# SCUT-CCNL/3DSIFT

Measured on AMD Instinct MI355X. Metric: Mvoxels/s end-to-end KpSiftAlgorithm on 512^3 fp32, higher is better.
Workload: dtype f32

## Files before the change

### 3dsift_amd/csrc/context.hip

```cpp
#include <float.h>
#include <math.h>
#include <stdlib.h>
#include <string.h>

#include <algorithm>
#include <atomic>
#include <mutex>
#include <thread>

#include "ctx_internal.h"

#pragma clang fp contract(off)

namespace s3d {

static thread_local std::string g_last_error;
void set_last_error(const std::string &s) { g_last_error = s; }

int set_device(int device) {
	int n = 0;
	if (hipGetDeviceCount(&n) != hipSuccess || n <= 0) {
		set_last_error("no HIP device visible: this library has no CPU fallback");
		return SIFT3D_ERR_NO_DEVICE;
	}
// ... 96 lines not shown
	}
}

extern "C" const char *sift3d_last_error(void) { return g_last_error.c_str(); }

extern "C" int sift3d_destroy(sift3d_handle c) {
	if (!c) return SIFT3D_OK;
	hipSetDevice(c->device);
	c->pending = false;
	if (c->uploader.joinable()) c->uploader.join();
	if (c->up_stream) { hipStreamSynchronize(c->up_stream); hipStreamDestroy(c->up_stream); c->up_stream = nullptr; }
	if (c->stream) hipStreamSynchronize(c->stream);
	if (c->own_stream && c->own_stream != c->stream) hipStreamSynchronize(c->own_stream);
	free_lists(c);
	if (!c->ext_arena) hipFree(c->arena);
	hipFree(c->in_own);
	hipFree(c->d_peer);
	hipFree(c->d_words);
	if (c->h_words) (void)hipHostFree(c->h_words);
	hipFree(c->d_slots_part);
	hipFree(c->det.masks); hipFree(c->det.block_counts); hipFree(c->det.block_offsets);
	hipFree(c->d_masks2); hipFree(c->d_counts2); hipFree(c->d_offsets2);
	if (c->ev_det_fork) hipEventDestroy(c->ev_det_fork);
	if (c->ev_det_join) hipEventDestroy(c->ev_det_join);
	if (c->ev_det_fork2) hipEventDestroy(c->ev_det_fork2);
	if (c->ev_det_join2) hipEventDestroy(c->ev_det_join2);
	hipFree(c->d_levels); hipFree(c->d_luts); hipFree(c->d_lutpool);
	for (auto &e : c->ev) if (e) hipEventDestroy(e);
	for (auto &e : c->ev_seed) if (e) hipEventDestroy(e);
	for (auto &e : c->ev_done) if (e) hipEventDestroy(e);
	if (c->ev_fork) hipEventDestroy(c->ev_fork);
	for (size_t o = 1; o < c->ostream.size(); o++) if (c->ostream[o] && c->ostream[o] != c->stream && c->ostream[o] != c->own_stream) hipStreamDestroy(c->ostream[o]);
	if (c->cstream) hipStreamDestroy(c->cstream);
	if (c->own_stream) hipStreamDestroy(c->own_stream);
	delete c;
	return SIFT3D_OK;
}

static int octaves_of(int nx, int ny, int nz) {
	const int mn = std::min(nx, std::min(ny, nz));
	return std::max(0, (int)log2f((float)mn) - 3 + 1);
}

void plan_pyramid(sift3d_ctx *c, int noct_total) {
	c->noct = noct_total >= 0 ? std::max(0, noct_total - c->octave_base) : octaves_of(c->nx, c->ny, c->nz);
	if (c->slab) c->noct = std::min(c->noct, 1);
	c->ng = c->p.num_kp_levels + 3;
	c->nd = c->p.num_kp_levels + 2;
	c->gss.assign((size_t)c->noct * c->ng, Level());
	c->dog.assign((size_t)c->noct * c->nd, Level());
	const double sigma0 = (double)c->p.sigma_default * pow(2.0, -1.0 / 3.0);
	for (int pyr = 0; pyr < 2; pyr++) {
		const int interval = pyr ? c->nd : c->ng;
		std::vector<Level> &P = pyr ? c->dog : c->gss;
		int nx = c->nx, ny = c->ny, nz = c->nz;
		float u = (float)(1 << c->octave_base);
		for (int o = 0; o < c->noct; o++) {
			for (int s = 0; s < interval; s++) {
				Level &L = P[(size_t)o * interval + s];
				L.nx = nx; L.ny = ny; L.nz = nz; L.unit = u;
				const double scale_factor = pow(2.0, (double)(o + c->octave_base) + (double)s / (double)c->p.num_kp_levels);
				L.scale = (float)(scale_factor * sigma0);
				if (c->slab) { L.bz = c->own1 - c->own0 + 2 * c->halo; L.zoff = c->own0 - c->halo; }
			}
			nx /= 2; ny /= 2; nz /= 2;
			u *= 2;
		}
	}
}

int upload_luts(sift3d_ctx *c, const std::vector<WinLut> &luts, std::vector<float> &pool) {
	if (pool.empty()) pool.push_back(-1.0f);
	if (c->d_luts) { S3D_HIP(hipFree(c->d_luts)); c->d_luts = nullptr; }
	if (c->d_lutpool) { S3D_HIP(hipFree(c->d_lutpool)); c->d_lutpool = nullptr; }
	S3D_HIP(hipMalloc(&c->d_luts, sizeof(WinLut) * luts.size()));
	S3D_HIP(hipMalloc(&c->d_lutpool, sizeof(float) * pool.size()));
	S3D_HIP(hipMemcpy(c->d_luts, luts.data(), sizeof(WinLut) * luts.size(), hipMemcpyHostToDevice));
	S3D_HIP(hipMemcpy(c->d_lutpool, pool.data(), sizeof(float) * pool.size(), hipMemcpyHostToDevice));
	return SIFT3D_OK;
}

std::vector<WinLut> blank_luts(const sift3d_ctx *c) {
	std::vector<WinLut> luts((size_t)std::max(1, c->noct + c->octave_base) * 8 * 2);
	for (auto &l : luts) { l.off = 0; l.len = 0; l.nin = -1; l.radius = 0; l.sigma = 0; l.fix_scale = 1.0f; l.wsum = 1.0f; l.list_off = -1; l.list_R = 0; }
	return luts;
}

static int build_luts(sift3d_ctx *c) {
	std::vector<WinLut> luts = blank_luts(c);
	std::vector<float> pool;
	for (int o = 0; o < c->noct; o++)
		for (int lv = 1; lv <= c->p.num_kp_levels && lv < 8; lv++) {
			const Level &D = c->dog[(size_t)o * c->nd + lv];
			const float u = D.unit, scale = D.scale;
			for (int which = 0; which < 2; which++) {
				float sigma, radius;
				if (which == 0) { sigma = 1.5f * scale; radius = sigma * 3.0f; }
				else { sigma = scale * 7.071067812f; radius = 2.0f * sigma; }
				if (!append_lut(pool, luts[((size_t)(o + c->octave_base) * 8 + lv) * 2 + which], which, sigma, radius, u, scale)) c->desc_lut_lds = false;
			}
		}
	return upload_luts(c, luts, pool);
}

static size_t al64(size_t n) { return (n + 63) & ~(size_t)63; }

size_t arena_floats_of(const sift3d_ctx *c) {
	size_t total = c->in_own ? 0 : al64(c->in.n());
	if (!c->slab) for (int o = 0; o < c->noct; o++) total += 2 * al64(c->gss[(size_t)o * c->ng].n());
	for (auto &L : c->gss) total += al64(L.n());
	for (auto &L : c->dog) total += al64(L.n());
	return total;
}

int create_common(sift3d_handle *out, const CreateCfg &cfg, const sift3d_params *params, int device) {
	*out = nullptr;
	if (cfg.nx <= 0 || cfg.ny <= 0 || cfg.nz <= 0) { set_last_error("bad dimensions"); return SIFT3D_ERR_ARG; }
	int rc = set_device(device);
	if (rc) return rc;
	sift3d_ctx *c = new sift3d_ctx();
	c->device = device;
	if (params) c->p = *params; else sift3d_default_params(&c->p);
	sift3d_default_detect_options(&c->dopt);
	if (c->p.num_kp_levels < 1 || c->p.num_kp_levels > 5) { delete c; set_last_error("num_kp_levels must be in [1,5]"); return SIFT3D_ERR_ARG; }
	c->nx = cfg.nx; c->ny = cfg.ny; c->nz = cfg.nz;
	c->octave_base = cfg.octave_base; c->seeded = cfg.seeded;
	c->slab = cfg.slab; c->own0 = cfg.z0; c->own1 = cfg.z1; c->halo = cfg.halo;
	c->use_fused = !hook(SIFT3D_HOOK_SEPARABLE);
	plan_pyramid(c, cfg.noct_total);
	c->in.nx = cfg.nx; c->in.ny = cfg.ny; c->in.nz = cfg.nz; c->in.unit = (float)(1 << c->octave_base); c->in.scale = 1.f;
	if (c->slab) { c->in.bz = c->own1 - c->own0 + 2 * c->halo; c->in.zoff = c->own0 - c->halo; }
	if (c->seeded) c->in.bz = 1;
	for (auto &L : c->gss) if ((size_t)L.nx * L.ny * L.planes() >= ((size_t)1 << 31)) { delete c; set_last_error("level too large for int32 voxel indices"); return SIFT3D_ERR_ARG; }

	std::vector<float> sig;
	float base_sigma;
	level_sigmas(c->p, sig, base_sigma);
	c->taps.resize(c->ng);
	bool ok = build_taps(base_sigma, c->base_taps);
	for (int i = 1; i < c->ng; i++) ok = ok && build_taps(sig[i], c->taps[i]);
	if (!ok) { delete c; set_last_error("Gaussian kernel wider than the supported 129 taps"); return SIFT3D_ERR_ARG; }

#define CHECKED(call) do { hipError_t e_ = (call); if (e_ != hipSuccess) { set_last_error(std::string(#call) + ": " + hipGetErrorString(e_)); sift3d_destroy(c); return SIFT3D_ERR_HIP; } } while (0)
	CHECKED(hipStreamCreateWithFlags(&c->stream, hipStreamNonBlocking));
	for (auto &e : c->ev) CHECKED(hipEventCreate(&e));
	CHECKED(hipEventCreateWithFlags(&c->ev_fork, hipEventDisableTiming));
	c->ostream.assign((size_t)std::max(1, c->noct), nullptr);
	c->ev_seed.assign(c->ostream.size(), nullptr);
	c->ev_done.assign(c->ostream.size(), nullptr);
	c->own_stream = c->stream;
	c->ostream[0] = c->stream;
	if (cfg.host_volume && !cfg.ext_arena && !c->slab && !c->seeded) {
		const size_t V0 = c->in.n();
		CHECKED(hipMalloc(&c->in_own, sizeof(float) * al64(V0)));
		CHECKED(hipStreamCreateWithFlags(&c->up_stream, hipStreamNonBlocking));
		const float *vol = cfg.host_volume;
		c->uploader = std::thread([c, vol, V0, device] {
			int r = set_device(device);
			if (r == SIFT3D_OK) r = staged_h2d(c->in_own, vol, sizeof(float) * V0, device, c->up_stream);
			if (r != SIFT3D_OK) c->upload_err = sift3d_last_error();
			c->upload_rc = r;
		});
	}
	const bool one_stream = hook(SIFT3D_HOOK_ONE_STREAM) != 0;
	for (size_t o = 0; o < c->ostream.size(); o++) {
		if (o > 0 && one_stream) c->ostream[o] = c->stream;
		else if (o > 0) {
// ... 734 lines not shown
```

### 3dsift_amd/csrc/kernels_orient.hip

```cpp
#include <float.h>

#include "sift3d_internal.h"

namespace s3d {

__device__ __forceinline__ float wave_sum(float v) {
#pragma unroll
	for (int o = 32; o > 0; o >>= 1) v = v + __shfl_xor(v, o, 64);
	return v;
}

__device__ __forceinline__ void win_bounds(float c, float rad, float u, int n, int &lo, int &hi) {
	int s = (int)floorf(c - __fdiv_rn(rad, u));
	lo = s > 1 ? s : 1;
	int e = (int)ceilf(c + __fdiv_rn(rad, u));
	hi = e < (n - 2) ? e : n - 2;
}

__device__ void eig_sym3(const double A[9], double w[3], double V[9]) {
	double a[9];
#pragma unroll
	for (int i = 0; i < 9; i++) { a[i] = A[i]; V[i] = (i % 4 == 0) ? 1.0 : 0.0; }
	for (int sweep = 0; sweep < 64; sweep++) {
		const double off = fabs(a[1]) + fabs(a[2]) + fabs(a[5]);
		const double diag = fabs(a[0]) + fabs(a[4]) + fabs(a[8]);
		if (off <= 1e-300 || off <= 1e-22 * diag) break;
#pragma unroll
		for (int pq = 0; pq < 3; pq++) {
			const int p = (pq == 2) ? 1 : 0, q = (pq == 0) ? 1 : 2;
			const double apq = a[3 * p + q];
			if (apq == 0.0) continue;
			const double theta = (a[4 * q] - a[4 * p]) / (2.0 * apq);
			const double t = (theta >= 0 ? 1.0 : -1.0) / (fabs(theta) + sqrt(theta * theta + 1.0));
			const double c = 1.0 / sqrt(t * t + 1.0), s = t * c;
#pragma unroll
			for (int k = 0; k < 3; k++) {
				const double akp = a[3 * k + p], akq = a[3 * k + q];
				a[3 * k + p] = c * akp - s * akq;
				a[3 * k + q] = s * akp + c * akq;
			}
#pragma unroll
			for (int k = 0; k < 3; k++) {
				const double apk = a[3 * p + k], aqk = a[3 * q + k];
				a[3 * p + k] = c * apk - s * aqk;
				a[3 * q + k] = s * apk + c * aqk;
			}
#pragma unroll
			for (int k = 0; k < 3; k++) {
				const double vkp = V[3 * k + p], vkq = V[3 * k + q];
				V[3 * k + p] = c * vkp - s * vkq;
				V[3 * k + q] = s * vkp + c * vkq;
			}
		}
	}
	w[0] = a[0]; w[1] = a[4]; w[2] = a[8];
#pragma unroll
	for (int j = 0; j < 3; j++) {
		const double n = sqrt(V[j] * V[j] + V[3 + j] * V[3 + j] + V[6 + j] * V[6 + j]);
		V[j] /= n; V[3 + j] /= n; V[6 + j] /= n;
	}
}

__device__ __forceinline__ float dot3f(const float *a, const float *b) { return a[0] * b[0] + a[1] * b[1] + a[2] * b[2]; }

__device__ int finish_orientation(DevKp &kp, const float T6[6], const float w3[3], float max_eig_ratio, float corner_thresh, bool *near = nullptr) {
	bool nr = false;
	float T[9] = {T6[0], T6[1], T6[2], T6[1], T6[3], T6[4], T6[2], T6[4], T6[5]};
#pragma unroll
	for (int i = 0; i < 9; i++) kp.st[i] = T[i];
	kp.win[0] = w3[0]; kp.win[1] = w3[1]; kp.win[2] = w3[2];
	const float gg = dot3f(w3, w3);
	nr = fabsf(gg - 1E-10f) <= 1E-13f;
	if (near) *near = nr;
	if (gg < 1E-10f) return -1;

	double A[9], wv[3], V[9];
#pragma unroll
	for (int i = 0; i < 9; i++) A[i] = (double)T[i];
	eig_sym3(A, wv, V);
	float val[3], vec[3][3];
#pragma unroll
	for (int j = 0; j < 3; j++) {
		val[j] = (float)wv[j];
		vec[j][0] = (float)V[j]; vec[j][1] = (float)V[3 + j]; vec[j][2] = (float)V[6 + j];
	}
#define S3D_CSWAP(i, j)                                                                   \
	if (val[j] < val[i]) {                                                                \
		float tv = val[i]; val[i] = val[j]; val[j] = tv;                                  \
		for (int c = 0; c < 3; c++) { float t2 = vec[i][c]; vec[i][c] = vec[j][c]; vec[j][c] = t2; } \
	}
	S3D_CSWAP(0, 1) S3D_CSWAP(1, 2) S3D_CSWAP(0, 1)
#undef S3D_CSWAP
#pragma unroll
	for (int j = 0; j < 3; j++) {
		kp.eigvalue[j] = val[j];
		kp.eigvector[3 * j] = vec[j][0]; kp.eigvector[3 * j + 1] = vec[j][1]; kp.eigvector[3 * j + 2] = vec[j][2];
	}
	const float r01 = fabsf(__fdiv_rn(val[0], val[1])), r12 = fabsf(__fdiv_rn(val[1], val[2]));
	nr = nr || fabsf(r01 - max_eig_ratio) <= 1e-4f || fabsf(r12 - max_eig_ratio) <= 1e-4f || !(r01 == r01) || !(r12 == r12);
	if (near) *near = nr;
	if (r01 > max_eig_ratio || r12 > max_eig_ratio) return -2;
	if ((double)fabsf(val[0] - val[1]) < DBL_EPSILON || (double)fabsf(val[0] - val[2]) < DBL_EPSILON ||
	    (double)fabsf(val[2] - val[1]) < DBL_EPSILON)
		return -2;

	const float d_norm = __fsqrt_rn(dot3f(w3, w3));
	float corner = FLT_MAX;
	for (int i = 2; i > 0; i--) {
		const float d = dot3f(vec[i], w3);
		const float q_norm = __fsqrt_rn(dot3f(vec[i], vec[i]));
		const float cos_ang = __fdiv_rn(d, d_norm * q_norm);
		const float a = fabsf(cos_ang);
		corner = corner < a ? corner : a;
		const float sgn = d > 0.0f ? 1.0f : -1.0f;
		vec[i][0] *= sgn; vec[i][1] *= sgn; vec[i][2] *= sgn;
	}
	nr = nr || fabsf(corner - corner_thresh) <= 1e-4f;
	if (near) *near = nr;
	if (corner < corner_thresh) return -3;
	if (near) *near = true;
	const float *v1 = vec[2], *v2 = vec[1];
	float vr[3];
	vr[0] = v1[1] * v2[2] - v1[2] * v2[1];
	vr[1] = v1[2] * v2[0] - v1[0] * v2[2];
	vr[2] = v1[0] * v2[1] - v1[1] * v2[0];
	kp.rot[0] = v1[0]; kp.rot[1] = v2[0]; kp.rot[2] = vr[0];
	kp.rot[3] = v1[1]; kp.rot[4] = v2[1]; kp.rot[5] = vr[1];
	kp.rot[6] = v1[2]; kp.rot[7] = v2[2]; kp.rot[8] = vr[2];
	return 1;
}

#ifndef S3D_ORI_UN
#define S3D_ORI_UN 2
#endif
constexpr int kTileW = 28, kTileH = 27;
constexpr int kTilePc = ((kTileW / 4) * kTileH + 63) / 64;
typedef float f4o __attribute__((ext_vector_type(4), aligned(4)));
constexpr int kOriLut = 256;

constexpr int kTermPitch = 68;
template <bool EXACT>
__global__ void __launch_bounds__(256) k_orient(DevKp *__restrict__ kps, int *__restrict__ codes, const unsigned *__restrict__ d_count, unsigned cap,
                                                const LevelRef *__restrict__ levels, const WinLut *__restrict__ luts,
                                                const float *__restrict__ lutpool, float max_eig, float corner, int part_rank,
                                                int part_world, const int *__restrict__ redo_list, const unsigned *__restrict__ redo_count) {
	__shared__ __attribute__((aligned(16))) float s_tile[4 * 3 * kTileW * kTileH];
	__shared__ float s_wlut[4 * kOriLut];
	__shared__ __attribute__((aligned(16))) float s_terms[EXACT ? 4 * 9 * kTermPitch : 4];
	const unsigned count = min(d_count[0], cap);
	const int lane = threadIdx.x & 63;
	const unsigned wave = blockIdx.x * (blockDim.x >> 6) + (threadIdx.x >> 6);
	const unsigned nwaves = gridDim.x * (blockDim.x >> 6);
	const unsigned pw = part_world > 1 ? (unsigned)part_world : 1u, pr = part_world > 1 ? (unsigned)part_rank : 0u;
	if (!EXACT && pw > 1)
		for (unsigned k = blockIdx.x * blockDim.x + threadIdx.x; k < count; k += gridDim.x * blockDim.x)
			if (k % pw != pr) { kps[k].code = 0; codes[k] = 0; }
	const unsigned owned = EXACT ? min(redo_count[0], cap) : (count > pr ? (count - pr + pw - 1) / pw : 0u);
	float *tb = &s_terms[EXACT ? (threadIdx.x >> 6) * 9 * kTermPitch : 0];
	for (unsigned j = wave; j < owned; j += nwaves) {
		const unsigned k = EXACT ? (unsigned)redo_list[j] : j * pw + pr;
		const int cxi = kps[k].x, cyi = kps[k].y, czi = kps[k].z;
		const int li = kps[k].octave * 8 + kps[k].level;
		const LevelRef L = levels[li];
		const WinLut lut = luts[li * 2 + 0];
		const float *__restrict__ wtab = lutpool + lut.off;
		const float u = L.unit, inv_u = __fdiv_rn(1.0f, u);
		int x0, x1, y0, y1, z0, z1;
		win_bounds((float)cxi, lut.radius, u, L.nx, x0, x1);
		win_bounds((float)cyi, lut.radius, u, L.ny, y0, y1);
		win_bounds((float)czi, lut.radius, u, L.nz, z0, z1);
		const int wx = x1 - x0 + 1, wy = y1 - y0 + 1;
		const int plane = (wx > 0 && wy > 0) ? wx * wy : 0;
		const float inv_wx = 1.0f / (float)(wx > 0 ? wx : 1);
		const size_t sy = (size_t)L.nx, sz = (size_t)L.nx * L.ny;
		const gfloat_p Ld = as_global(L.d);
		float t00 = 0.f, t01 = 0.f, t02 = 0.f, t11 = 0.f, t12 = 0.f, t22 = 0.f, g0 = 0.f, g1 = 0.f, g2 = 0.f;
		float chain = 0.f;
		auto emit = [&](bool ok, float c1p, float c1m, float c2p, float c2m, float c3p, float c3m, float ww, int nvalid) {
			float vx = 0.5f * (c1p - c1m);
			float vy = 0.5f * (c2p - c2m);
			float vz = 0.5f * (c3p - c3m);
			vx = vx * inv_u; vy = vy * inv_u; vz = vz * inv_u;
			if (!EXACT) {
				if (ok) {
					const float wx = vx * ww, wy = vy * ww, wz = vz * ww;
					t00 = __fmaf_rn(vx, wx, t00);
					t01 = __fmaf_rn(vx, wy, t01);
					t02 = __fmaf_rn(vx, wz, t02);
					t11 = __fmaf_rn(vy, wy, t11);
					t12 = __fmaf_rn(vy, wz, t12);
					t22 = __fmaf_rn(vz, wz, t22);
					g0 = g0 + wx; g1 = g1 + wy; g2 = g2 + wz;
				}
			} else {
				tb[0 * kTermPitch + lane] = ok ? vx * vx * ww : 0.0f;
				tb[1 * kTermPitch + lane] = ok ? vx * vy * ww : 0.0f;
				tb[2 * kTermPitch + lane] = ok ? vx * vz * ww : 0.0f;
				tb[3 * kTermPitch + lane] = ok ? vy * vy * ww : 0.0f;
				tb[4 * kTermPitch + lane] = ok ? vy * vz * ww : 0.0f;
				tb[5 * kTermPitch + lane] = ok ? vz * vz * ww : 0.0f;
				tb[6 * kTermPitch + lane] = ok ? vx * ww : 0.0f;
				tb[7 * kTermPitch + lane] = ok ? vy * ww : 0.0f;
				tb[8 * kTermPitch + lane] = ok ? vz * ww : 0.0f;
				__builtin_amdgcn_fence(__ATOMIC_RELEASE, "wavefront");
				__builtin_amdgcn_wave_barrier();
				__builtin_amdgcn_fence(__ATOMIC_ACQUIRE, "wavefront");
				if (lane < 9) {
					const float4 *row = reinterpret_cast<const float4 *>(tb + lane * kTermPitch);
#pragma unroll
					for (int h = 0; h < 2; h++) {
						if (h * 32 >= nvalid) break;
						float4 v[8];
#pragma unroll
						for (int i = 0; i < 8; i++) v[i] = row[h * 8 + i];
#pragma unroll
						for (int i = 0; i < 8; i++) { chain = chain + v[i].x; chain = chain + v[i].y; chain = chain + v[i].z; chain = chain + v[i].w; }
					}
				}
				__builtin_amdgcn_wave_barrier();
			}
		};
		const int tw = wx + 2, th = wy + 2;
		if (plane > 0 && z1 >= z0 && tw <= kTileW && th <= kTileH && lut.len <= kOriLut) {
			float *tile = &s_tile[(threadIdx.x >> 6) * 3 * kTileW * kTileH];
			float *wl = &s_wlut[(threadIdx.x >> 6) * kOriLut];
			for (int i = lane; i < lut.len && i < kOriLut; i += 64) wl[i] = wtab[i];
			const int npx = (tw + 3) >> 2;
			const int tnp = npx * th;
			const float inv_npx = 1.0f / (float)npx;
			int toff[kTilePc];
			int goff[kTilePc];
#pragma unroll
			for (int i = 0; i < kTilePc; i++) {
				const int idx = lane + 64 * i;
				const int ty = (int)(((float)idx + 0.5f) * inv_npx);
				const int px = idx - ty * npx;
				const bool ok = idx < tnp;
				toff[i] = ok ? ty * kTileW + 4 * px : -1;
				goff[i] = ok ? (x0 - 1 + 4 * px) + (int)sy * (y0 - 1 + ty) : (x0 - 1) + (int)sy * (y0 - 1);
			}
			const gfloat_p base = Ld - sz * (size_t)L.zoff;
			f4o pf[kTilePc];
			auto request = [&](int zp) {
				const gfloat_p pl = base + sz * (size_t)zp;
#pragma unroll
				for (int i = 0; i < kTilePc; i++) pf[i] = *reinterpret_cast<const f4o __attribute__((address_space(1))) *>(pl + goff[i]);
			};
			auto deposit = [&](int slot) {
				float *dstp = tile + slot * (kTileW * kTileH);
#pragma unroll
				for (int i = 0; i < kTilePc; i++)
					if (toff[i] >= 0) *reinterpret_cast<float4 *>(dstp + toff[i]) = make_float4(pf[i].x, pf[i].y, pf[i].z, pf[i].w);
			};
			request(z0 - 1); deposit(0);
			request(z0);     deposit(1);
			request(z0 + 1);
			int sm = 0, sc = 1, sp = 2;
			constexpr int kEL = 8;
			const unsigned *__restrict__ lst = reinterpret_cast<const unsigned *>(lutpool) + (lut.list_off >= 0 ? lut.list_off : 0);
			const int LR = lut.list_R;
			const unsigned *__restrict__ ent = lst + 2 * LR + 2;
			const bool use_list = lut.list_off >= 0 && (int)lst[LR + 1] - (int)lst[LR] <= 64 * kEL;
			const int ox = cxi - x0 - 128, oy = cyi - y0 - 128;
			unsigned En[kEL];
			int cntn = 0;
			auto fetch_entries = [&](int dzp) {
				const int pi = dzp + LR;
				const bool has = use_list && pi >= 0 && pi <= 2 * LR;
				const int e0 = has ? (int)lst[pi] : 0, e1 = has ? (int)lst[pi + 1] : 0;
				cntn = e1 - e0;
#pragma unroll
				for (int i = 0; i < kEL; i++) {
					const int idx = e0 + i * 64 + lane;
					En[i] = ent[idx < e1 ? idx : e0];
				}
			};
			fetch_entries(z0 - czi);
			for (int z = z0; z <= z1; z++) {
#if !defined(S3D_ODIAG) || !(S3D_ODIAG & 2)
				deposit(sp);
				request(min(z + 2, z1 + 1));
#endif
				__builtin_amdgcn_fence(__ATOMIC_RELEASE, "wavefront");
				__builtin_amdgcn_wave_barrier();
				__builtin_amdgcn_fence(__ATOMIC_ACQUIRE, "wavefront");
				const float *pm = tile + sm * (kTileW * kTileH), *pc = tile + sc * (kTileW * kTileH), *pp = tile + sp * (kTileW * kTileH);
				const int dz = z - czi;
				constexpr int kUn = S3D_ORI_UN;
#ifdef S3D_ODIAG
				if (S3D_ODIAG & 1) { } else
#endif
				if (use_list) {
					unsigned E[kEL];
#pragma unroll
					for (int i = 0; i < kEL; i++) E[i] = En[i];
					const int cnt = cntn;
					fetch_entries(dz + 1);
#pragma unroll
					for (int p0 = 0; p0 < kEL; p0 += kUn) {
						if (p0 * 64 >= cnt) break;
						float nb[kUn][6], w[kUn];
#pragma unroll
						for (int q = 0; q < kUn; q++) {
							const unsigned e = E[p0 + q];
							const int lx = (int)(e & 255u) + ox, ly = (int)((e >> 8) & 255u) + oy;
							const bool ok = (p0 + q) * 64 + lane < cnt && (unsigned)lx < (unsigned)wx && (unsigned)ly < (unsigned)wy;
							w[q] = ok ? wl[e >> 16] : -1.0f;
							const int o = ok ? __mul24(ly + 1, kTileW) + lx + 1 : kTileW + 1;
							nb[q][0] = pc[o + 1]; nb[q][1] = pc[o - 1]; nb[q][2] = pc[o + kTileW]; nb[q][3] = pc[o - kTileW];
							nb[q][4] = pp[o]; nb[q][5] = pm[o];
						}
#pragma unroll
						for (int q = 0; q < kUn; q++) {
							if (EXACT && (p0 + q) * 64 >= cnt) break;
							emit(!(w[q] < 0.0f), nb[q][0], nb[q][1], nb[q][2], nb[q][3], nb[q][4], nb[q][5], w[q], min(64, cnt - (p0 + q) * 64));
						}
					}
				} else if (EXACT) {
					for (int vb = 0; vb < plane; vb += 64) {
						const int v = vb + lane;
						const int ly = (int)(((float)v + 0.5f) * inv_wx);
						const int lx = v - ly * wx;
						const int dx = x0 + lx - cxi, dy = y0 + ly - cyi;
						const int n = dx * dx + dy * dy + dz * dz;
						const bool in = v < plane && n < lut.len;
						const float ww = in ? wl[n] : -1.0f;
						const int o = in ? __mul24(ly + 1, kTileW) + lx + 1 : kTileW + 1;
						emit(!(ww < 0.0f), pc[o + 1], pc[o - 1], pc[o + kTileW], pc[o - kTileW], pp[o], pm[o], ww, min(64, plane - vb));
					}
				} else
				for (int v0 = lane; v0 < plane; v0 += 64 * kUn) {
					float nb[kUn][6], w[kUn];
#pragma unroll
					for (int q = 0; q < kUn; q++) {
						const int v = v0 + 64 * q;
						const int ly = (int)(((float)v + 0.5f) * inv_wx);
						const int lx = v - ly * wx;
						const int dx = x0 + lx - cxi, dy = y0 + ly - cyi;
						const int n = dx * dx + dy * dy + dz * dz;
						const bool ok = v < plane && n < lut.len;
						w[q] = ok ? wl[n] : -1.0f;
						const int o = ok ? __mul24(ly + 1, kTileW) + lx + 1 : kTileW + 1;
						nb[q][0] = pc[o + 1]; nb[q][1] = pc[o - 1]; nb[q][2] = pc[o + kTileW]; nb[q][3] = pc[o - kTileW];
						nb[q][4] = pp[o]; nb[q][5] = pm[o];
					}
#pragma unroll
					for (int q = 0; q < kUn; q++)
						emit(!(w[q] < 0.0f), nb[q][0], nb[q][1], nb[q][2], nb[q][3], nb[q][4], nb[q][5], w[q], 64);
				}
				__builtin_amdgcn_wave_barrier();
				const int tmp = sm; sm = sc; sc = sp; sp = tmp;
			}
		} else
		for (int z = z0; z <= z1; z++) {
			const int dz = z - czi;
			for (int vb = 0; vb < plane; vb += 64) {
				const int v = vb + lane;
				const int ly = (int)(((float)v + 0.5f) * inv_wx);
				const int lx = v - ly * wx;
				const int x = x0 + lx, y = y0 + ly;
// ... 202 lines not shown
```

### 3dsift_amd/csrc/sift3d_internal.h

```cpp
#pragma once

#include <hip/hip_runtime.h>
#include <stdint.h>

#include <string>
#include <vector>

#include "../../include/sift3d_hip.h"
#include "../../include/sift3d_hip_test.h"

#pragma clang fp contract(off)

namespace s3d {

#ifndef S3D_MAX_HW
#define S3D_MAX_HW 64
#endif
constexpr int kMaxHW = S3D_MAX_HW;
constexpr int kMaxTaps = 2 * kMaxHW + 1;
constexpr int kDesc = SIFT3D_DESC_NUMEL;
constexpr int kFaces = 20;

struct Taps {
	int hw;
	float w[kMaxTaps];
};

struct EdgeFrac {
	float f[3][kMaxHW + 1];
};

struct ZRange {
	int nz;
	int zoff;
	int nzg;
	int zo0, zo1;
};
inline ZRange whole(int nz) { return ZRange{nz, 0, nz, 0, nz}; }

struct Level {
	float *d = nullptr;
	int nx = 0, ny = 0, nz = 0;
	float unit = 1.f;
	float scale = 0.f;
	int bz = 0;
	int zoff = 0;
	int planes() const { return bz ? bz : nz; }
	size_t n() const { return (size_t)nx * ny * planes(); }
	ZRange zr(int zo0, int zo1) const { return ZRange{planes(), zoff, nz, zo0, zo1}; }
	ZRange zr_all() const { return ZRange{planes(), zoff, nz, 0, planes()}; }
};

struct DevKp {
	int x, y, z;
	int octave, level;
	float scale;
	int code;
	int slot;
	float win[3];
	float eigvalue[3];
	float eigvector[9];
	float rot[9];
	float st[9];
};

struct FaceConst {
	float e1[3], e2[3], t[3], q[3];
	float qe2;
	int idx[3];
	float centre[3];
};

struct WinLut {
	int off;
	int len;
	int nin;
	float radius;
	float sigma;
	float fix_scale;
	float wsum;
	int list_off, list_R;
};
constexpr int kMaxDescLut = 1536;

struct FaceSym {
	int face[32];
	int vert[32][3];
	int slot[32][3];
};

void launch_absmax(const float *src, size_t n, unsigned *d_max_bits, hipStream_t st, unsigned *d_nonfinite = nullptr);
void launch_scale_by_max(float *data, size_t n, const unsigned *d_max_bits, hipStream_t st);
void launch_dog_from_gss(const float *hi, const float *lo, float *dog, size_t n, hipStream_t st);
void launch_conv_axis(int axis, const float *src, float *dst, int nx, int ny, int nz, const Taps &t,
                      const float *prev, float *dog, unsigned *d_dogmax, hipStream_t st, bool exact = false);
struct MarchHalf { float *d = nullptr; int nx = 0, ny = 0, nz = 0; };
bool march_half_ok(int nx, int ny, const ZRange &zr);
bool march_applicable(int nx, int ny, int nzg, const Taps &t);
bool launch_march_level(const float *src, float *dst, float *dog, unsigned *dogmax, int nx, int ny, const ZRange &zr, const Taps &t,
                        hipStream_t st, int plan_slots = 0, int prio = 0, const MarchHalf *half = nullptr);
void launch_copy16(const float *src, float *dst, size_t nfloats, hipStream_t st);
constexpr int kCopySegs = 32, kMaxMergePtrs = 16;
struct CopySegs { const float *src[kCopySegs]; float *dst[kCopySegs]; size_t floats[kCopySegs]; int n = 0; };
struct MaxMerge { const float *in[kMaxMergePtrs]; float *out[kMaxMergePtrs]; int nin = 0, nout = 0, n = 0; };
void launch_copy_segments(const CopySegs &a, hipStream_t st);
void launch_max_merge(const MaxMerge &a, hipStream_t st);
constexpr int kSmallMaxOct = 4, kSmallMaxLv = 8;
struct SmallOct { float *g[kSmallMaxLv]; float *dog[kSmallMaxLv]; int nx, ny, nz; };
struct SmallArgs {
	SmallOct oct[kSmallMaxOct];
	int noct, ng, nd, seed;
	unsigned build_mask, dog_mask;
	unsigned *dogmax;
	int hwp;
	float w[kSmallMaxLv][9];
	const float *parent;
	int pnx, pny;
};
bool small_octave_fits(int nx, int ny, int nz, int max_hw);
int small_padded_hw(int max_hw);
void launch_small_octaves(const SmallArgs &a, hipStream_t st);
void launch_downsample(const float *src, int snx, int sny, float *dst, int nx, int ny, int nz, hipStream_t st);

struct DetectBufs {
	unsigned long long *masks;
	unsigned *block_counts;
	unsigned *block_offsets;
	unsigned *total;
	unsigned *prov = nullptr;
	unsigned *prov_count = nullptr;
	unsigned prov_cap = 0;
};
constexpr int kMaxKpLevels = 5;
struct DetectLevels {
	const float *cur[kMaxKpLevels], *prev[kMaxKpLevels], *next[kMaxKpLevels];
	const float *prev0_hi, *prev0_lo;
	const float *nextl_hi, *nextl_lo;
	int nextl_slot;
	const float *lazy_src;
	const unsigned *absmax_bits[kMaxKpLevels];
	int level_id[kMaxKpLevels];
	float scale[kMaxKpLevels];
};
constexpr int kLazySlots = 52;
struct DetectOpts {
	int neighbours = 8, refine = 0;
	float max_offset = 0.5f, contrast_thresh = 0.0f, edge_ratio = 0.0f;
};
void launch_detect_mark(const DetectLevels &L, int nlevels, int nx, int ny, const ZRange &zr, float peak_thresh, int octave,
                        const DetectBufs &b, hipStream_t st, const Taps *lazy_taps, const DetectOpts *opt = nullptr);
void launch_mark_full(const DetectLevels &L, int nlevels, int nx, int ny, const ZRange &zr, int rows, float peak_thresh, const DetectOpts &opt,
                      const DetectBufs &b, hipStream_t st);
constexpr int kDogTabOct = 12, kDogTabLv = 8;
struct DogTable {
	const float *d[kDogTabOct][kDogTabLv];
	int nx[kDogTabOct], ny[kDogTabOct];
	int octave_base;
};
void launch_detect_emit(const DetectLevels &L, int nlevels, int nx, int ny, const ZRange &zr, int octave, const DetectBufs &b, DevKp *out,
                        unsigned cap, hipStream_t st);
struct DetectEmitItem { const DetectLevels *L; int nlevels, nx, ny; ZRange zr; int octave; const DetectBufs *b; };
void launch_detect_emit_multi(const DetectEmitItem *items, int n, DevKp *out, unsigned cap, unsigned *total, hipStream_t st);
void launch_detect_octave(const DetectLevels &L, int nlevels, int nx, int ny, const ZRange &zr, float peak_thresh, int octave,
                          const DetectBufs &b, DevKp *out, unsigned cap, hipStream_t st, const Taps *lazy_taps = nullptr);

// ... 131 lines not shown
```

### 3dsift_amd/csrc/tables.hip

```cpp
#include <float.h>
#include <math.h>
#include <stdlib.h>
#include <string.h>

#include <algorithm>
#include <atomic>
#include <mutex>
#include <thread>

#include "ctx_internal.h"

#pragma clang fp contract(off)

namespace s3d {

bool build_taps(float sigma, Taps &t) {
	sigma = sigma > 0 ? sigma : 0;
	int hw = 1;
	if (sigma > 0) {
		hw = (int)ceil((double)sigma * 3.0);
		if (hw < 1) hw = 1;
	}
	if (hw > kMaxHW) return false;
	t.hw = hw;
// ... 23 lines not shown
	}
	base_sigma = sqrtf(sig[0] * sig[0] - p.sigma_n_default * p.sigma_n_default);
}

static void cross3(const float *a, const float *b, float *o) {
	o[0] = a[1] * b[2] - a[2] * b[1];
	o[1] = a[2] * b[0] - a[0] * b[2];
	o[2] = a[0] * b[1] - a[1] * b[0];
}
static float dot3(const float *a, const float *b) { return a[0] * b[0] + a[1] * b[1] + a[2] * b[2]; }

void build_faces(FaceConst *F) {
	const double gr = 1.6180339887;
	const double vert[12][3] = {{0, 1, gr}, {0, -1, gr}, {0, 1, -gr}, {0, -1, -gr}, {1, gr, 0}, {-1, gr, 0},
	                            {1, -gr, 0}, {-1, -gr, 0}, {gr, 0, 1}, {-gr, 0, 1}, {gr, 0, -1}, {-gr, 0, -1}};
	static const int faces[kFaces][3] = {{0, 1, 8}, {0, 8, 4}, {0, 4, 5}, {0, 5, 9}, {0, 9, 1}, {1, 6, 8}, {8, 6, 10},
	                                     {8, 10, 4}, {4, 10, 2}, {4, 2, 5}, {5, 2, 11}, {5, 11, 9}, {9, 11, 7}, {9, 7, 1},
	                                     {1, 7, 6}, {3, 6, 7}, {3, 7, 11}, {3, 11, 2}, {3, 2, 10}, {3, 10, 6}};
	for (int f = 0; f < kFaces; f++) {
		float v[3][3];
		for (int j = 0; j < 3; j++) {
			F[f].idx[j] = faces[f][j];
			float raw[3] = {(float)vert[faces[f][j]][0], (float)vert[faces[f][j]][1], (float)vert[faces[f][j]][2]};
			const double mag = (double)sqrtf(dot3(raw, raw));
			const double sca = 1.0 / mag;
			for (int c = 0; c < 3; c++) v[j][c] = (float)((double)raw[c] * sca);
		}
		float a[3], b[3], n[3];
		for (int c = 0; c < 3; c++) { a[c] = v[2][c] - v[1][c]; b[c] = v[1][c] - v[0][c]; }
		cross3(a, b, n);
		if (dot3(n, v[0]) < 0)
			for (int c = 0; c < 3; c++) std::swap(v[0][c], v[1][c]);
		for (int c = 0; c < 3; c++) {
			F[f].e1[c] = v[1][c] - v[0][c];
			F[f].e2[c] = v[2][c] - v[0][c];
			F[f].t[c] = (float)((double)v[0][c] * (-1.0));
		}
		cross3(F[f].t, F[f].e1, F[f].q);
		F[f].qe2 = dot3(F[f].q, F[f].e2);
		for (int c = 0; c < 3; c++) F[f].centre[c] = (v[0][c] + v[1][c] + v[2][c]) / 3.0f;
	}
}

bool build_facesym(const FaceConst *F, FaceSym *S) {
	const double gr = 1.6180339887, nrm = sqrt(1.0 + gr * gr);
	for (int type = 0; type < 4; type++)
		for (int bits = 0; bits < 8; bits++) {
			const double sx = (bits & 1) ? -1.0 : 1.0, sy = (bits & 2) ? -1.0 : 1.0, sz = (bits & 4) ? -1.0 : 1.0;
			const double A[3] = {0, sy, sz * gr}, B[3] = {sx, sy * gr, 0}, C[3] = {sx * gr, 0, sz};
			const double Am[3] = {0, -sy, sz * gr}, Bm[3] = {-sx, sy * gr, 0}, Cm[3] = {sx * gr, 0, -sz};
			const double *role[3];
			switch (type) {
			case 0: role[0] = A; role[1] = B; role[2] = C; break;
			case 1: role[0] = C; role[1] = Cm; role[2] = B; break;
			case 2: role[0] = A; role[1] = Am; role[2] = C; break;
			default: role[0] = B; role[1] = Bm; role[2] = A; break;
			}
			int found = -1, slot[3] = {-1, -1, -1};
			for (int f = 0; f < kFaces && found < 0; f++) {
				double v[3][3];
				for (int c = 0; c < 3; c++) { v[0][c] = -(double)F[f].t[c]; v[1][c] = v[0][c] + (double)F[f].e1[c]; v[2][c] = v[0][c] + (double)F[f].e2[c]; }
				int sl[3] = {-1, -1, -1}, hit = 0;
				for (int r = 0; r < 3; r++)
					for (int j = 0; j < 3; j++) {
						double d = 0;
						for (int c = 0; c < 3; c++) d += fabs(v[j][c] - role[r][c] / nrm);
						if (d < 1e-4) { sl[r] = j; hit++; }
					}
				if (hit == 3 && sl[0] != sl[1] && sl[1] != sl[2] && sl[0] != sl[2]) { found = f; for (int r = 0; r < 3; r++) slot[r] = sl[r]; }
			}
			if (found < 0) return false;
			const int key = type * 8 + bits;
			S->face[key] = found;
			for (int r = 0; r < 3; r++) { S->slot[key][r] = slot[r]; S->vert[key][r] = F[found].idx[slot[r]]; }
		}
	return true;
}


bool append_lut(std::vector<float> &pool, WinLut &L, int which, float sigma, float radius, float u, float scale) {
	bool fits_lds = true;
	const float r2 = radius * radius, uu = u * u;
	const int len = (int)floor((double)r2 / (double)uu) + 2;
	L.off = (int)pool.size(); L.len = len; L.nin = -1; L.radius = radius; L.sigma = sigma; L.fix_scale = 1.0f; L.list_off = -1; L.list_R = 0;
	if (which == 1) {
		const double cw = 5.0 * (double)scale / (double)u, bound = (cw + 2.0) * (cw + 2.0) * (cw + 2.0) * 1.7321 * 1.001;
		int k = (int)floor(log2(2147483647.0 / bound));
		k = std::max(0, std::min(k, 29));
		L.fix_scale = (float)ldexp(1.0, k);
	}
	if (which == 1 && len > kMaxDescLut) fits_lds = false;
	for (int n = 0; n < len; n++) {
		const float sq = (float)n * uu;
		float w;
		if (!(sq > r2)) L.nin = n;
		if (sq > r2) w = -1.0f;
		else if (which == 0) w = expf((float)(-0.5 * (double)sq / (double)(sigma * sigma)));
		else w = expf(-0.5f * sq / (sigma * sigma)) * (0.5f / u);
		pool.push_back(w);
	}
	const int R = (int)floor(sqrt((double)std::max(L.nin, 0)));
	double ws = 0.0;
	for (int dz = -R; dz <= R; dz++)
		for (int dy = -R; dy <= R; dy++)
			for (int dx = -R; dx <= R; dx++) {
				const int n = dx * dx + dy * dy + dz * dz;
				if (n <= L.nin) ws += (double)pool[(size_t)L.off + n] * (which == 1 ? (double)u / 0.5 : 1.0);
			}
	L.wsum = (float)std::max(ws, 1.0);
	if (which == 0 && R <= 127 && L.nin < 65536) {
		std::vector<unsigned> words((size_t)2 * R + 2);
		for (int dz = -R; dz <= R; dz++) {
			words[(size_t)(dz + R)] = (unsigned)(words.size() - ((size_t)2 * R + 2));
			for (int dy = -R; dy <= R; dy++)
				for (int dx = -R; dx <= R; dx++) {
					const int n = dx * dx + dy * dy + dz * dz;
					if (n <= L.nin) words.push_back((unsigned)(dx + 128) | (unsigned)(dy + 128) << 8 | (unsigned)n << 16);
				}
		}
		words[(size_t)2 * R + 1] = (unsigned)(words.size() - ((size_t)2 * R + 2));
		L.list_off = (int)pool.size(); L.list_R = R;
		pool.resize(pool.size() + words.size());
		memcpy(pool.data() + L.list_off, words.data(), words.size() * sizeof(unsigned));
	}
	return fits_lds;
}

}
```

Before: 19430.

## Add fast orientation path with precomputed per-plane offset/weight entry lists

Builds, on the host, per-z-plane lists of (byte offset into the LDS tile, Gaussian weight) pairs for the orientation window, padded to wavefront multiples. When the window fits fully inside the volume, the orient kernel uses these lists to read gradient neighbours straight from the tile, with no per-voxel index decoding or weight lookups. Scaling by 0.5/u is deferred to the end. The change also forces keypoint fields to be scalar via readfirstlane and adds an occupancy hint to the launch bounds, at the cost of more code, extra table memory and small rounding differences in the non-exact path.

```diff
diff --git a/3dsift_amd/csrc/context.hip b/3dsift_amd/csrc/context.hip
--- a/3dsift_amd/csrc/context.hip
+++ b/3dsift_amd/csrc/context.hip
@@ -202,7 +202,7 @@
 
 std::vector<WinLut> blank_luts(const sift3d_ctx *c) {
 	std::vector<WinLut> luts((size_t)std::max(1, c->noct + c->octave_base) * 8 * 2);
-	for (auto &l : luts) { l.off = 0; l.len = 0; l.nin = -1; l.radius = 0; l.sigma = 0; l.fix_scale = 1.0f; l.wsum = 1.0f; l.list_off = -1; l.list_R = 0; }
+	for (auto &l : luts) { l.off = 0; l.len = 0; l.nin = -1; l.radius = 0; l.sigma = 0; l.fix_scale = 1.0f; l.wsum = 1.0f; l.list_off = -1; l.list_R = 0; l.fl_off = -1; l.fl_ent = 0; }
 	return luts;
 }
 
diff --git a/3dsift_amd/csrc/kernels_orient.hip b/3dsift_amd/csrc/kernels_orient.hip
--- a/3dsift_amd/csrc/kernels_orient.hip
+++ b/3dsift_amd/csrc/kernels_orient.hip
@@ -1,4 +1,6 @@
 #include <float.h>
+
+#include <type_traits>
 
 #include "sift3d_internal.h"
 
@@ -133,14 +135,15 @@
 #ifndef S3D_ORI_UN
 #define S3D_ORI_UN 2
 #endif
-constexpr int kTileW = 28, kTileH = 27;
+constexpr int kTileW = kOriTileW, kTileH = 27;
 constexpr int kTilePc = ((kTileW / 4) * kTileH + 63) / 64;
 typedef float f4o __attribute__((ext_vector_type(4), aligned(4)));
+typedef unsigned u2o __attribute__((ext_vector_type(2)));
 constexpr int kOriLut = 256;
 
 constexpr int kTermPitch = 68;
 template <bool EXACT>
-__global__ void __launch_bounds__(256) k_orient(DevKp *__restrict__ kps, int *__restrict__ codes, const unsigned *__restrict__ d_count, unsigned cap,
+__global__ void __launch_bounds__(256, EXACT ? 3 : 4) k_orient(DevKp *__restrict__ kps, int *__restrict__ codes, const unsigned *__restrict__ d_count, unsigned cap,
                                                 const LevelRef *__restrict__ levels, const WinLut *__restrict__ luts,
                                                 const float *__restrict__ lutpool, float max_eig, float corner, int part_rank,
                                                 int part_world, const int *__restrict__ redo_list, const unsigned *__restrict__ redo_count) {
@@ -159,8 +162,8 @@
 	float *tb = &s_terms[EXACT ? (threadIdx.x >> 6) * 9 * kTermPitch : 0];
 	for (unsigned j = wave; j < owned; j += nwaves) {
 		const unsigned k = EXACT ? (unsigned)redo_list[j] : j * pw + pr;
-		const int cxi = kps[k].x, cyi = kps[k].y, czi = kps[k].z;
-		const int li = kps[k].octave * 8 + kps[k].level;
+		const int cxi = __builtin_amdgcn_readfirstlane(kps[k].x), cyi = __builtin_amdgcn_readfirstlane(kps[k].y), czi = __builtin_amdgcn_readfirstlane(kps[k].z);
+		const int li = __builtin_amdgcn_readfirstlane(kps[k].octave * 8 + kps[k].level);
 		const LevelRef L = levels[li];
 		const WinLut lut = luts[li * 2 + 0];
 		const float *__restrict__ wtab = lutpool + lut.off;
@@ -176,6 +179,24 @@
 		const gfloat_p Ld = as_global(L.d);
 		float t00 = 0.f, t01 = 0.f, t02 = 0.f, t11 = 0.f, t12 = 0.f, t22 = 0.f, g0 = 0.f, g1 = 0.f, g2 = 0.f;
 		float chain = 0.f;
+		auto chain_add = [&](int nvalid) {
+			__builtin_amdgcn_fence(__ATOMIC_RELEASE, "wavefront");
+			__builtin_amdgcn_wave_barrier();
+			__builtin_amdgcn_fence(__ATOMIC_ACQUIRE, "wavefront");
+			if (lane < 9) {
+				const float4 *row = reinterpret_cast<const float4 *>(tb + lane * kTermPitch);
+#pragma unroll
+				for (int h = 0; h < 2; h++) {
+					if (h * 32 >= nvalid) break;
+					float4 v[8];
+#pragma unroll
+					for (int i = 0; i < 8; i++) v[i] = row[h * 8 + i];
+#pragma unroll
+					for (int i = 0; i < 8; i++) { chain = chain + v[i].x; chain = chain + v[i].y; chain = chain + v[i].z; chain = chain + v[i].w; }
+				}
+			}
+			__builtin_amdgcn_wave_barrier();
+		};
 		auto emit = [&](bool ok, float c1p, float c1m, float c2p, float c2m, float c3p, float c3m, float ww, int nvalid) {
 			float vx = 0.5f * (c1p - c1m);
 			float vy = 0.5f * (c2p - c2m);
@@ -202,22 +223,7 @@
 				tb[6 * kTermPitch + lane] = ok ? vx * ww : 0.0f;
 				tb[7 * kTermPitch + lane] = ok ? vy * ww : 0.0f;
 				tb[8 * kTermPitch + lane] = ok ? vz * ww : 0.0f;
-				__builtin_amdgcn_fence(__ATOMIC_RELEASE, "wavefront");
-				__builtin_amdgcn_wave_barrier();
-				__builtin_amdgcn_fence(__ATOMIC_ACQUIRE, "wavefront");
-				if (lane < 9) {
-					const float4 *row = reinterpret_cast<const float4 *>(tb + lane * kTermPitch);
-#pragma unroll
-					for (int h = 0; h < 2; h++) {
-						if (h * 32 >= nvalid) break;
-						float4 v[8];
-#pragma unroll
-						for (int i = 0; i < 8; i++) v[i] = row[h * 8 + i];
-#pragma unroll
-						for (int i = 0; i < 8; i++) { chain = chain + v[i].x; chain = chain + v[i].y; chain = chain + v[i].z; chain = chain + v[i].w; }
-					}
-				}
-				__builtin_amdgcn_wave_barrier();
+				chain_add(nvalid);
 			}
 		};
 		const int tw = wx + 2, th = wy + 2;
@@ -275,7 +281,98 @@
 					En[i] = ent[idx < e1 ? idx : e0];
 				}
 			};
+			const unsigned *__restrict__ fh = reinterpret_cast<const unsigned *>(lutpool) + (lut.fl_off >= 0 ? lut.fl_off : 0);
+			typedef const u2o __attribute__((address_space(1))) *gent_p;
+			const gent_p fe = (gent_p)(lutpool + lut.fl_ent);
+			const bool fast = lut.fl_off >= 0 && 2 * LR < 64 && (int)fh[2 * LR + 1] <= 64 * kEL &&
+			                  x0 <= cxi - LR && x1 >= cxi + LR && y0 <= cyi - LR && y1 >= cyi + LR && z0 <= czi - LR && z1 >= czi + LR;
+			if (fast) {
+				constexpr int kPl = kTileW * kTileH;
+				const char *cb = reinterpret_cast<const char *>(tile + (cyi - y0) * kTileW + (cxi - x0 + 1));
+				u2o Fn[kEL];
+				int fcntn = 0, frealn = 0;
+				const u2o head = ((gent_p)fh)[lane <= 2 * LR ? lane : 0];
+				auto fetch_fast = [&](int dzp) {
+					const int pi = dzp + LR;
+					const bool has = pi >= 0 && pi <= 2 * LR;
+					const int pl = has ? pi : 0;
+					const int e0 = has ? __builtin_amdgcn_readlane((int)head.x, pl) : 0;
+					frealn = has ? __builtin_amdgcn_readlane((int)head.y, pl) : 0;
+					fcntn = (frealn + 63) & ~63;
+					const gent_p src = fe + e0 + lane;
+#pragma unroll
+					for (int i = 0; i < kEL / 2; i++) Fn[i] = src[i * 64];
+					if (fcntn > 64 * (kEL / 2)) {
+#pragma unroll
+						for (int i = kEL / 2; i < kEL; i++) Fn[i] = src[i * 64];
+					}
+				};
+				auto plane_fast = [&](auto rot, int z) {
+					constexpr int sm_ = decltype(rot)::value % 3, sc_ = (decltype(rot)::value + 1) % 3, sp_ = (decltype(rot)::value + 2) % 3;
+					deposit(sp_);
+					request(min(z + 2, z1 + 1));
+					__builtin_amdgcn_fence(__ATOMIC_RELEASE, "wavefront");
+					__builtin_amdgcn_wave_barrier();
+					__builtin_amdgcn_fence(__ATOMIC_ACQUIRE, "wavefront");
+					u2o F[kEL];
+#pragma unroll
+					for (int i = 0; i < kEL; i++) F[i] = Fn[i];
+					const int cnt = fcntn, real = frealn;
+					fetch_fast(z - czi + 1);
+#pragma unroll
+					for (int p = 0; p < kEL; p++) {
+						if (p * 64 >= (EXACT ? real : cnt)) break;
+						const char *a = cb + (int)F[p].x;
+						const float ww = __uint_as_float(F[p].y);
+						auto rd = [&](int slot, int d) { return *reinterpret_cast<const float *>(a + (slot * kPl + kTileW + d) * (int)sizeof(float)); };
+						const float c1p = rd(sc_, 1), c1m = rd(sc_, -1), c2p = rd(sc_, kTileW), c2m = rd(sc_, -kTileW), c3p = rd(sp_, 0), c3m = rd(sm_, 0);
+						if (!EXACT) {
+							const float vx = c1p - c1m, vy = c2p - c2m, vz = c3p - c3m;
+							const float wx = vx * ww, wy = vy * ww, wz = vz * ww;
+							t00 = __fmaf_rn(vx, wx, t00);
+							t01 = __fmaf_rn(vx, wy, t01);
+							t02 = __fmaf_rn(vx, wz, t02);
+							t11 = __fmaf_rn(vy, wy, t11);
+							t12 = __fmaf_rn(vy, wz, t12);
+							t22 = __fmaf_rn(vz, wz, t22);
+							g0 = g0 + wx; g1 = g1 + wy; g2 = g2 + wz;
+						} else {
+							const bool ok = ww != 0.0f;
+							float vx = 0.5f * (c1p - c1m);
+							float vy = 0.5f * (c2p - c2m);
+							float vz = 0.5f * (c3p - c3m);
+							vx = vx * inv_u; vy = vy * inv_u; vz = vz * inv_u;
+							vx = ok ? vx : 0.0f; vy = ok ? vy : 0.0f; vz = ok ? vz : 0.0f;
+							tb[0 * kTermPitch + lane] = vx * vx * ww;
+							tb[1 * kTermPitch + lane] = vx * vy * ww;
+							tb[2 * kTermPitch + lane] = vx * vz * ww;
+							tb[3 * kTermPitch + lane] = vy * vy * ww;
+							tb[4 * kTermPitch + lane] = vy * vz * ww;
+							tb[5 * kTermPitch + lane] = vz * vz * ww;
+							tb[6 * kTermPitch + lane] = vx * ww;
+							tb[7 * kTermPitch + lane] = vy * ww;
+							tb[8 * kTermPitch + lane] = vz * ww;
+							chain_add(min(64, real - p * 64));
+						}
+					}
+					__builtin_amdgcn_wave_barrier();
+				};
+				fetch_fast(z0 - czi);
+				for (int z = z0; z <= z1; z += 3) {
+					plane_fast(std::integral_constant<int, 0>(), z);
+					if (z + 1 > z1) break;
+					plane_fast(std::integral_constant<int, 1>(), z + 1);
+					if (z + 2 > z1) break;
+					plane_fast(std::integral_constant<int, 2>(), z + 2);
+				}
+				if (!EXACT) {
+					const float s1 = 0.5f * inv_u, s2 = s1 * s1;
+					t00 *= s2; t01 *= s2; t02 *= s2; t11 *= s2; t12 *= s2; t22 *= s2;
+					g0 *= s1; g1 *= s1; g2 *= s1;
+				}
+			} else
 			fetch_entries(z0 - czi);
+			if (!fast)
 			for (int z = z0; z <= z1; z++) {
 #if !defined(S3D_ODIAG) || !(S3D_ODIAG & 2)
 				deposit(sp);
diff --git a/3dsift_amd/csrc/sift3d_internal.h b/3dsift_amd/csrc/sift3d_internal.h
--- a/3dsift_amd/csrc/sift3d_internal.h
+++ b/3dsift_amd/csrc/sift3d_internal.h
@@ -80,7 +80,10 @@
 	float fix_scale;
 	float wsum;
 	int list_off, list_R;
-};
+	int fl_off, fl_ent;
+};
+constexpr int kOriTileW = 28;
+constexpr int kOriListLanes = 8;
 constexpr int kMaxDescLut = 1536;
 
 struct FaceSym {
diff --git a/3dsift_amd/csrc/tables.hip b/3dsift_amd/csrc/tables.hip
--- a/3dsift_amd/csrc/tables.hip
+++ b/3dsift_amd/csrc/tables.hip
@@ -129,7 +129,7 @@
 	bool fits_lds = true;
 	const float r2 = radius * radius, uu = u * u;
 	const int len = (int)floor((double)r2 / (double)uu) + 2;
-	L.off = (int)pool.size(); L.len = len; L.nin = -1; L.radius = radius; L.sigma = sigma; L.fix_scale = 1.0f; L.list_off = -1; L.list_R = 0;
+	L.off = (int)pool.size(); L.len = len; L.nin = -1; L.radius = radius; L.sigma = sigma; L.fix_scale = 1.0f; L.list_off = -1; L.list_R = 0; L.fl_off = -1; L.fl_ent = 0;
 	if (which == 1) {
 		const double cw = 5.0 * (double)scale / (double)u, bound = (cw + 2.0) * (cw + 2.0) * (cw + 2.0) * 1.7321 * 1.001;
 		int k = (int)floor(log2(2147483647.0 / bound));
@@ -169,6 +169,35 @@
 		L.list_off = (int)pool.size(); L.list_R = R;
 		pool.resize(pool.size() + words.size());
 		memcpy(pool.data() + L.list_off, words.data(), words.size() * sizeof(unsigned));
+		std::vector<unsigned> head((size_t)2 * (2 * R + 1));
+		std::vector<unsigned> ents;
+		auto push = [&](int off, float w) {
+			unsigned wb;
+			memcpy(&wb, &w, sizeof wb);
+			ents.push_back((unsigned)off); ents.push_back(wb);
+		};
+		for (int dz = -R; dz <= R; dz++) {
+			const size_t first = ents.size() / 2;
+			for (int dy = -R; dy <= R; dy++)
+				for (int dx = -R; dx <= R; dx++) {
+					const int n = dx * dx + dy * dy + dz * dz;
+					if (n <= L.nin) push((dy * kOriTileW + dx) * (int)sizeof(float), pool[(size_t)L.off + n]);
+				}
+			head[(size_t)2 * (dz + R)] = (unsigned)first;
+			head[(size_t)2 * (dz + R) + 1] = (unsigned)(ents.size() / 2 - first);
+			while ((ents.size() / 2) % 64) push(0, 0.0f);
+		}
+		for (int i = 0; i < 64 * kOriListLanes; i++) push(0, 0.0f);
+		bool positive = true;
+		for (int n = 0; n <= L.nin; n++) positive = positive && pool[(size_t)L.off + n] > 0.0f;
+		if (!positive) return fits_lds;
+		if (pool.size() % 2) pool.push_back(0.0f);
+		L.fl_off = (int)pool.size();
+		pool.resize(pool.size() + head.size());
+		memcpy(pool.data() + L.fl_off, head.data(), head.size() * sizeof(unsigned));
+		L.fl_ent = (int)pool.size();
+		pool.resize(pool.size() + ents.size());
+		memcpy(pool.data() + L.fl_ent, ents.data(), ents.size() * sizeof(unsigned));
 	}
 	return fits_lds;
 }
```

Result: faster. 19710, median of 6 (+1.4%).
